# lc700x/desktop2stereo

Hardware: AMD Instinct MI355X
Metric: stereo frames/sec @1080p DepthAnything-v2-ViT-B (higher is better)
Workload: dtype bf16; 1 GPU; DepthAnything-v2-vitb bf16, 1920x1080 uint8 RGB noise frames, batch 1 per GPU, Depth Resolution 518 (model input 294x518), Full-SBS uint8 output 3840x1080, pred; parallelism=frame-sharded dp1, no data-path collective (each rank generates its own frames)

## Files before the change

desktop2stereo_amd/csrc/engine.hip:

```cpp
#include <map>
#include <string>
#include <vector>
#include <cmath>
#include <cstring>

#include "gemm.h"
#include "linear_site.h"
#include "vit_ops.h"

using namespace d2s;

namespace {

struct HostT { std::vector<float> data; std::vector<int64_t> shape; };

struct PackedW {
    void* w = nullptr;
    float* bias = nullptr;
    int N = 0, K = 0, Kpad = 0;
};

struct Layer {
    float *ln1g, *ln1b, *ln2g, *ln2b, *ls1, *ls2;
    PackedW qkv, proj, fc1, fc2;
    PackedW w8[4];
    std::vector<float> sw[4];
    PackedW qkv_ln, fc1_ln;
    float *csum_qkv = nullptr, *csum_fc1 = nullptr;
    float* deq[4] = {nullptr, nullptr, nullptr, nullptr};
    PackedW w8_ln[2];
    std::vector<float> sw_ln[2];
    float *csum8[2] = {nullptr, nullptr}, *deq_ln[2] = {nullptr, nullptr};
};

constexpr int NSITE = 6;

}

struct d2s_engine {
    d2s_model_desc d;
    int device = 0;
    int prec = D2S_PREC_BF16;
    int wprec = D2S_PREC_BF16;
    std::map<std::string, HostT> host;
    bool finalized = false;
    int h = 0, w = 0, gh = 0, gw = 0, P = 0, N = 0, Npad = 0, maxB = 0;
    uint64_t bytes = 0;
    std::vector<void*> allocs;

    PackedW patch;
    float *cls = nullptr, *pos = nullptr;
    std::vector<Layer> L;
    float *lnfg = nullptr, *lnfb = nullptr;
    struct { PackedW proj, resize, conv; PackedW proj_ln; float* csum = nullptr; } re[4];
    struct { PackedW proj, r1c1, r1c2, r2c1, r2c2; } fu[4];
    PackedW head1, head2;
    float* w3 = nullptr;
    float b3 = 0.f;

    float* resid = nullptr;
    void *lnbuf = nullptr, *qkv = nullptr, *vt = nullptr, *attn = nullptr, *mlp = nullptr, *patchA = nullptr;
    void* tapbuf[4] = {nullptr, nullptr, nullptr, nullptr};
    void* rproj[4] = {nullptr, nullptr, nullptr, nullptr};
    void* rres[4] = {nullptr, nullptr, nullptr, nullptr};
    void* feat[4] = {nullptr, nullptr, nullptr, nullptr};
    int fH[4], fW[4];
    void* scr[5] = {nullptr, nullptr, nullptr, nullptr, nullptr};
    float* splitk_ws = nullptr;
    size_t splitk_elems = 0;
    hipStream_t side = nullptr;
    hipEvent_t ev_tap[4] = {nullptr, nullptr, nullptr, nullptr}, ev_ln[4] = {nullptr, nullptr, nullptr, nullptr}, ev_side = nullptr;
    int tap_slots = 0;
    bool overlap = true;
    float* splitk_ws_side = nullptr;
    void* r1[3] = {nullptr, nullptr, nullptr};
    void* r1tmp = nullptr;
    struct TMod {
        int C = 0, sites = 0;
        float *gn_g = nullptr, *gn_b = nullptr;
        float *ln_g[2] = {nullptr, nullptr}, *ln_b[2] = {nullptr, nullptr}, *ffn_g = nullptr, *ffn_b = nullptr;
        PackedW proj_in, proj_out, kvq[2], to_out[2], ff1, ff2;
        float* ptab[2] = {nullptr, nullptr};
        void* cache[2] = {nullptr, nullptr};
        size_t ring_bytes = 0;
        PackedW kvq_ln[2], ff1_ln;
        float *csum_kvq[2] = {nullptr, nullptr}, *csum_ff1 = nullptr;
    } tm[4];
    float* tm_stats = nullptr;
    bool tm_fold = false;
    struct TSlot { int head = 0, filled = 0; };
    std::vector<TSlot> tm_slot;
    int row_ids[D2S_MAX_STREAMS] = {0};
    float* tm_hs = nullptr;
    void *tm_a = nullptr, *tm_kv = nullptr, *tm_u = nullptr, *tm_g = nullptr, *tm_out = nullptr;
    float *pre_x = nullptr, *depth_small = nullptr, *depth_post = nullptr;
    void* post_ws = nullptr;
    uint64_t post_ws_bytes = 0;
    float* ema_state = nullptr;
    int ema_init = 0;
    std::vector<int> ema_slot_init;
    bool taps = false;
    float* tap_hidden = nullptr;
    int last_batch = 0;
    bool fp8 = false, fp8_ready = false, calib = false;
    bool lnf = false;
    bool no_lnfuse = false;
    bool attn_prescaled = false;
    float* lnstats = nullptr;
    float* amax = nullptr;
    std::vector<float> act_scale;
    struct ProfRec { int cls; double flops, bytes; hipEvent_t a, b; };
    bool prof_on = false;
    std::vector<ProfRec> prof_recs;
    std::vector<hipEvent_t> prof_pool;
    size_t prof_used = 0;
};

namespace {

int dev_alloc(d2s_engine* e, void** p, size_t bytes, bool zero = false) {
    if (bytes == 0) bytes = 16;
    D2S_HIP(hipMalloc(p, bytes));
    e->allocs.push_back(*p);
    e->bytes += bytes;
    if (zero) D2S_HIP(hipMemset(*p, 0, bytes));
    return D2S_OK;
}

int dev_upload(d2s_engine* e, void** p, const void* host, size_t bytes) {
    int rc = dev_alloc(e, p, bytes);
    if (rc) return rc;
    D2S_HIP(hipMemcpy(*p, host, bytes, hipMemcpyHostToDevice));
    return D2S_OK;
}

#define RC(x) do { int _rc = (x); if (_rc != D2S_OK) return _rc; } while (0)

enum { PC_GEMM = 0, PC_CONV, PC_ATTN, PC_LN, PC_ELT, PC_PRE, PC_POST, PC_WARP, PC_N };
const char* const PC_NAMES[PC_N] = {"gemm_linear", "gemm_conv3x3", "attention", "layernorm", "elementwise", "preprocess",
                                    "post_process", "stereo_warp"};

hipEvent_t prof_event(d2s_engine* e) {
    if (e->prof_used == e->prof_pool.size()) { hipEvent_t ev; (void)hipEventCreate(&ev); e->prof_pool.push_back(ev); }
    return e->prof_pool[e->prof_used++];
}
void prof_begin(d2s_engine* e, int cls, double flops, double bytes, hipStream_t st) {
    if (!e->prof_on) return;
    d2s_engine::ProfRec r; r.cls = cls; r.flops = flops; r.bytes = bytes; r.a = prof_event(e); r.b = prof_event(e);
    (void)hipEventRecord(r.a, st);
    e->prof_recs.push_back(r);
}
void prof_end(d2s_engine* e, hipStream_t st) {
    if (!e->prof_on) return;
    (void)hipEventRecord(e->prof_recs.back().b, st);
}
#define PROF(cls, fl, by, call) do { prof_begin(e, cls, fl, by, st); int _rc = (call); prof_end(e, st); if (_rc != D2S_OK) return _rc; } while (0)

const HostT* find(d2s_engine* e, const std::string& name) {
    auto it = e->host.find(name);
    if (it == e->host.end()) { set_error("missing weight tensor: " + name); return nullptr; }
    return &it->second;
}

int upload_f32(d2s_engine* e, const std::string& name, size_t n, float** out) {
    const HostT* t = find(e, name);
    if (!t) return D2S_E_MISSING;
    if (t->data.size() != n) { set_error("weight " + name + ": wrong element count"); return D2S_E_MISSING; }
    return dev_upload(e, (void**)out, t->data.data(), n * sizeof(float));
}

int upload_linear(d2s_engine* e, LinearImage im, PackedW& out, float** csum = nullptr, std::vector<float>* sw = nullptr) {
    RC(dev_upload(e, &out.w, im.w.data(), im.w.size()));
    out.N = im.N; out.K = im.K; out.Kpad = im.Kpad;
    out.bias = nullptr;
    if (!im.bias.empty()) RC(dev_upload(e, (void**)&out.bias, im.bias.data(), im.bias.size() * sizeof(float)));
    if (csum) {
        D2S_REQUIRE(!im.csum.empty(), "upload_linear: a colsum was asked for, but no LayerNorm is folded into this linear");
        RC(dev_upload(e, (void**)csum, im.csum.data(), im.csum.size() * sizeof(float)));
    }
    if (sw) *sw = std::move(im.sw);
    return D2S_OK;
}

int pack_linear(d2s_engine* e, const std::string& wname, const std::string& bname, int N, int K, PackedW& out) {
    const HostT* w = find(e, wname);
    if (!w) return D2S_E_MISSING;
    if (w->data.size() != (size_t)N * K) { set_error("weight " + wname + ": wrong shape"); return D2S_E_MISSING; }
    const float* b = nullptr;
    if (!bname.empty()) { const HostT* bt = find(e, bname); if (!bt || bt->data.size() != (size_t)N) { set_error("bad bias " + bname); return D2S_E_MISSING; } b = bt->data.data(); }
    const float* p = w->data.data();
    return upload_linear(e, prepare_linear(e->wprec, N, K, [&](int n, int k) { return p[(size_t)n * K + k]; }, b), out);
}

int pack_conv3(d2s_engine* e, const std::string& wname, const std::string& bname, int Co, int Ci, PackedW& out) {
    const HostT* w = find(e, wname);
    if (!w) return D2S_E_MISSING;
    if (w->data.size() != (size_t)Co * Ci * 9) { set_error("weight " + wname + ": wrong shape"); return D2S_E_MISSING; }
    const float* b = nullptr;
    if (!bname.empty()) { const HostT* bt = find(e, bname); if (!bt || bt->data.size() != (size_t)Co) { set_error("bad bias " + bname); return D2S_E_MISSING; } b = bt->data.data(); }
    const float* p = w->data.data();
    return upload_linear(e, prepare_linear(e->wprec, Co, 9 * Ci, [&](int n, int k) { return p[conv3_weight_index(n, k, Ci)]; }, b), out);
}

int pack_convT(d2s_engine* e, const std::string& wname, const std::string& bname, int C, int ks, PackedW& out) {
    const HostT* w = find(e, wname);
    const HostT* bt = find(e, bname);
    if (!w || !bt) return D2S_E_MISSING;
    if (w->data.size() != (size_t)C * C * ks * ks || bt->data.size() != (size_t)C) { set_error("weight " + wname + ": wrong shape"); return D2S_E_MISSING; }
    const float* p = w->data.data();
    int N = ks * ks * C;
    std::vector<float> bias(N);
    for (int n = 0; n < N; ++n) bias[n] = bt->data[n % C];
    return upload_linear(e, prepare_linear(e->wprec, N, C, [&](int n, int k) { return p[convT_weight_index(n, k, C, ks)]; }, bias.data()), out);
}

void cubic_coeffs(float t, float c[4]) {
    const float A = -0.75f;
    auto c1 = [&](float x) { return ((A + 2.f) * x - (A + 3.f)) * x * x + 1.f; };
    auto c2 = [&](float x) { return ((A * x - 5.f * A) * x + 8.f * A) * x - 4.f * A; };
    c[0] = c2(t + 1.f); c[1] = c1(t); c[2] = c1(1.f - t); c[3] = c2(2.f - t);
}

void interp_pos(const float* pos, int grid, int D, int gh, int gw, std::vector<float>& out, double offset = 0.0) {
    out.assign((size_t)(1 + gh * gw) * D, 0.f);
    std::memcpy(out.data(), pos, D * sizeof(float));
    if (gh == grid && gw == grid) { std::memcpy(out.data() + D, pos + D, (size_t)grid * grid * D * sizeof(float)); return; }
    float sy = (float)grid / (float)gh, sx = (float)grid / (float)gw;
    if (offset != 0.0) {
        sy = (float)(1.0 / (((double)gh + offset) / (double)grid)); sx = (float)(1.0 / (((double)gw + offset) / (double)grid));
    }
    for (int oy = 0; oy < gh; ++oy) {
        float fy = sy * ((float)oy + 0.5f) - 0.5f;
        float iyf = floorf(fy);
        float cy[4]; cubic_coeffs(fy - iyf, cy);
        int iy = (int)iyf;
        for (int ox = 0; ox < gw; ++ox) {
            float fx = sx * ((float)ox + 0.5f) - 0.5f;
            float ixf = floorf(fx);
            float cx[4]; cubic_coeffs(fx - ixf, cx);
            int ix = (int)ixf;
            float* o = out.data() + (size_t)(1 + oy * gw + ox) * D;
            for (int d = 0; d < D; ++d) {
                float acc = 0.f;
                for (int a = 0; a < 4; ++a) {
                    int yy = std::min(std::max(iy - 1 + a, 0), grid - 1);
                    float row = 0.f;
                    for (int b = 0; b < 4; ++b) {
                        int xx = std::min(std::max(ix - 1 + b, 0), grid - 1);
                        row += pos[(size_t)(1 + yy * grid + xx) * D + d] * cx[b];
                    }
                    acc += row * cy[a];
                }
                o[d] = acc;
            }
        }
    }
}

GemmA plainA(const void* p, long lda) { GemmA a = {}; a.ptr = p; a.mode = A_PLAIN; a.lda = lda; return a; }
GemmA splitA(const void* p, long lda, bool split) { GemmA a = plainA(p, lda); a.bx3 = split ? 1 : 0; return a; }
GemmA convA(const void* p, int Hi, int Wi, int C, int Ho, int Wo, int stride, int relu) {
    GemmA a = {}; a.ptr = p; a.mode = A_CONV3; a.Hi = Hi; a.Wi = Wi; a.C = C; a.Ho = Ho; a.Wo = Wo; a.stride = stride; a.relu = relu; return a;
}

int gemm(d2s_engine* e, const GemmA& a, const PackedW& w, int M, const GemmEpi& ep, hipStream_t st) {
    int Kl = w.K % (e->prec == D2S_PREC_BF16 ? 8 : 4) ? w.Kpad : w.K;
    GemmEpi ep2 = ep;
    if (ep.map == MAP_ROWS) {
        ep2.part = (e->side && st == e->side) ? e->splitk_ws_side : e->splitk_ws;
        ep2.part_elems = e->splitk_elems;
    }
    PROF(a.mode == A_CONV3 ? PC_CONV : PC_GEMM, 2.0 * M * w.N * w.K, 0, launch_gemm(e->wprec, 0, a, w.w, M, w.N, Kl, w.Kpad, ep2, st));
    return D2S_OK;
}

int gemm8(d2s_engine* e, const GemmA& a, const PackedW& w, int M, const GemmEpi& ep, hipStream_t st) {
    PROF(PC_GEMM, 2.0 * M * w.N * w.K, 0, launch_gemm(D2S_PREC_FP8_OPERANDS, 0, a, w.w, M, w.N, w.K, w.Kpad, ep, st));
    return D2S_OK;
}

int conv3(d2s_engine* e, const void* in, int B, int Hi, int Wi, int C, int stride, int relu_in, const PackedW& w,
          void* out, int act, const void* res1, const void* res2, hipStream_t st) {
    int Ho = (Hi + 2 - 3) / stride + 1, Wo = (Wi + 2 - 3) / stride + 1;
    GemmA a = convA(in, Hi, Wi, C, Ho, Wo, stride, relu_in);
    GemmEpi ep = rowsE(out, OUT_T, w.N, w.bias);
    ep.act = act; ep.res1 = res1; ep.res2 = res2;
    return gemm(e, a, w, B * Ho * Wo, ep, st);
}

void window_rows(const d2s_engine::TSlot& sl, bool fold, void* ring, AttnRow& attn, CacheRow& store) {
    const bool in_attn = fold && sl.filled;
    attn = AttnRow{ring, (int16_t)sl.head, (int16_t)(sl.filled ? 32 : 1), in_attn ? sl.head : -1};
    store = CacheRow{ring, sl.filled ? sl.head : 0, sl.filled ? (in_attn ? 0 : 1) : 31};
}

int run_temporal(d2s_engine* e, int m, const void* x, void* out, int B, hipStream_t st, const void* add = nullptr) {
    d2s_engine::TMod& t = e->tm[m];
    const int C = t.C, S = B * t.sites, prec = e->prec;
    const int* ids = e->row_ids;
    const bool fold = e->tm_fold;
    int slots = 0;
    auto producer = [&](GemmEpi& ep) { if (fold) epi_ln_producer(ep, e->tm_a, e->tm_stats, &slots); };
    auto consumer = [&](GemmEpi& ep, const float* csum) { epi_ln_consumer(ep, e->tm_stats, slots, csum, 1e-5f, C); };
    void* gn_out = fold ? e->tm_out : e->tm_a;
    PROF(PC_ELT, 0, 0, launch_groupnorm(prec, x, t.gn_g, t.gn_b, gn_out, t.sites, C, 32, 1e-6f, st, B));
    {
        GemmEpi ep = rowsE(e->tm_hs, OUT_F32, C, t.proj_in.bias);
        producer(ep);
        RC(gemm(e, plainA(gn_out, C), t.proj_in, S, ep, st));
    }
    for (int a = 0; a < 2; ++a) {
        const bool folded = fold && slots >= 1 && slots <= 16;
        if (!folded) PROF(PC_LN, 0, 0, launch_layernorm(prec, e->tm_hs, t.ln_g[a], t.ln_b[a], e->tm_a, S, C, 1e-5f, 0, 0, 0, st));
        {
            GemmEpi ep = rowsE(e->tm_kv, OUT_T, 3 * C, folded ? t.kvq_ln[a].bias : nullptr);
            if (folded) consumer(ep, t.csum_kvq[a]);
            RC(gemm(e, plainA(e->tm_a, C), folded ? t.kvq_ln[a] : t.kvq[a], S, ep, st));
        }
        AttnRows attn = {};
        CacheRows store = {};
        double win_rows = 0;
        bool store_due = false;
        for (int r = 0; r < B; ++r) {
            window_rows(e->tm_slot[ids[r]], fold, (char*)t.cache[a] + (size_t)ids[r] * t.ring_bytes, attn.r[r], store.r[r]);
            win_rows += attn.r[r].Tw;
            store_due |= store.r[r].nslots > 0;
        }
        PROF(PC_ATTN, 4.0 * t.sites * win_rows * C, 0, launch_temporal_attn(prec, e->tm_kv, t.ptab[a], e->tm_out, t.sites, C, 31, B, attn, st));
        {
            GemmEpi ep = epi_residual(e->tm_hs, C, t.to_out[a].bias, nullptr);
            producer(ep);
            RC(gemm(e, plainA(e->tm_out, C), t.to_out[a], S, ep, st));
        }
        if (store_due) PROF(PC_ELT, 0, 0, launch_cache_store(prec, e->tm_kv, t.sites, C, B, store, st));
    }
    {
        const bool folded = fold && slots >= 1 && slots <= 16;
        if (!folded) PROF(PC_LN, 0, 0, launch_layernorm(prec, e->tm_hs, t.ffn_g, t.ffn_b, e->tm_a, S, C, 1e-5f, 0, 0, 0, st));
        if (folded) {
            GemmEpi ep = rowsE(e->tm_g, OUT_T, 4 * C, t.ff1_ln.bias);
            ep.act = ACT_GEGLU;
            consumer(ep, t.csum_ff1);
            RC(gemm(e, plainA(e->tm_a, C), t.ff1_ln, S, ep, st));
        } else {
            GemmEpi ep = rowsE(e->tm_u, OUT_T, 8 * C, t.ff1.bias);
            RC(gemm(e, plainA(e->tm_a, C), t.ff1, S, ep, st));
            PROF(PC_ELT, 0, 0, launch_geglu(prec, e->tm_u, e->tm_g, S, 4 * C, st));
        }
    }
    {
        GemmEpi ep = epi_residual(e->tm_hs, C, t.ff2.bias, nullptr);
        if (fold) epi_ln_producer(ep, e->tm_a, nullptr, nullptr);
        RC(gemm(e, plainA(e->tm_g, 4 * C), t.ff2, S, ep, st));
    }
    const void* a_out = e->tm_a;
    if (!fold) {
        if (prec == D2S_PREC_BF16) PROF(PC_ELT, 0, 0, launch_cast_f32(prec, e->tm_hs, e->tm_a, (long)S * C, st));
        else a_out = e->tm_hs;
    }
    {
        GemmEpi ep = rowsE(out, OUT_T, C, t.proj_out.bias);
        ep.res1 = x; ep.res2 = add;
        RC(gemm(e, plainA(a_out, C), t.proj_out, S, ep, st));
    }
    return D2S_OK;
}

int neck_proj(d2s_engine* e, int i, int B, hipStream_t st, bool fold) {
    const d2s_model_desc& d = e->d;
    const int D = d.hidden, Mp = B * e->P, c = d.neck[i];
    if (!fold) return gemm(e, plainA(e->tapbuf[i], D), e->re[i].proj, Mp, rowsE(e->rproj[i], OUT_T, c, e->re[i].proj.bias), st);
    GemmEpi ep = rowsE(e->rproj[i], OUT_T, c, e->re[i].proj_ln.bias);
    epi_ln_consumer(ep, e->lnstats, e->tap_slots, e->re[i].csum, d.ln_eps, D);
    const int skip = epi_tap_fold_rows(ep, B, e->N, e->P);
    return gemm(e, plainA((const bf16_t*)e->lnbuf + (size_t)skip * D, D), e->re[i].proj_ln, skip ? Mp : B * e->N, ep, st);
}

int neck_rest(d2s_engine* e, int i, int B, hipStream_t st) {
    const d2s_model_desc& d = e->d;
    const int F = d.fusion, gh = e->gh, gw = e->gw, Mp = B * e->P, c = d.neck[i];
    const void* src = e->rproj[i];
    int Hs = gh, Ws = gw;
    if (i < 2) {
        int ks = i == 0 ? 4 : 2;
        RC(gemm(e, plainA(e->rproj[i], c), e->re[i].resize, Mp, epi_convT(e->rres[i], c, e->re[i].resize.bias, gh, gw, ks), st));
        src = e->rres[i]; Hs = gh * ks; Ws = gw * ks;
    } else if (i == 3) {
        RC(conv3(e, e->rproj[i], B, gh, gw, c, 2, 0, e->re[i].resize, e->rres[i], ACT_NONE, nullptr, nullptr, st));
        src = e->rres[i]; Hs = (gh - 1) / 2 + 1; Ws = (gw - 1) / 2 + 1;
    }
    if (d.temporal && i == 2) { RC(run_temporal(e, 0, src, e->rres[2], B, st)); src = e->rres[2]; }
    if (d.temporal && i == 3) { RC(run_temporal(e, 1, src, e->scr[0], B, st)); src = e->scr[0]; }
    RC(conv3(e, src, B, Hs, Ws, c, 1, 0, e->re[i].conv, e->feat[i], ACT_NONE, nullptr, nullptr, st));
    if (i < 3) {
        const int idx = 3 - i;
        RC(conv3(e, e->feat[i], B, Hs, Ws, F, 1, 1, e->fu[idx].r1c1, e->r1tmp, ACT_NONE, nullptr, nullptr, st));
        RC(conv3(e, e->r1tmp, B, Hs, Ws, F, 1, 1, e->fu[idx].r1c2, e->r1[i], ACT_NONE, e->feat[i], nullptr, st));
    }
    return D2S_OK;
}

int forward(d2s_engine* e, const float* x, float* depth, int B, hipStream_t st) {
    const d2s_model_desc& d = e->d;
    const int D = d.hidden, N = e->N, P = e->P, M = B * N, Mp = B * P, prec = e->prec;
    const int F = d.fusion;
    const PrecRules pr = prec_rules(d.precision);
    const bool use_side = e->overlap && e->side != nullptr && !e->prof_on;
    if (e->fp8 && !e->fp8_ready && !e->calib) {
        set_error("D2S_PREC_FP8 engine: activation scales are not set, call d2s_engine_calibrate first");
        return D2S_E_STATE;
    }
    if (x) PROF(PC_ELT, 0, 0, launch_patchify(prec, x, e->patchA, B, e->h, e->w, d.patch, e->patch.Kpad, e->cls, e->pos, e->resid, N, D, st));
    {
        RC(gemm(e, plainA(e->patchA, e->patch.Kpad), e->patch, Mp, epi_patch_embed(e->resid, D, e->patch.bias, e->pos, P, N), st));
    }
    if (e->taps) D2S_HIP(hipMemcpyAsync(e->tap_hidden, e->resid, (size_t)N * D * 4, hipMemcpyDeviceToDevice, st));
    int tap_i = 0;
    const bool f8 = e->fp8 && !e->calib;
    const bool f8a = f8 && pr.e4m3_attn;
    const bool x3 = e->wprec == D2S_PREC_BF16X3;
    static EnvInt lnf_pp{"D2S_LNF_PP", 1};
    const bool pp_fold = lnf_pp.get() && e->lnf && e->wprec == D2S_PREC_BF16 && !e->calib && !e->taps && D % 256 == 0 && D <= 1024 &&
                         gemm_pp_min_tiles() > 0 && (long)cdiv(M, 256) * (D / 256) >= gemm_pp_min_tiles();
    const bool lnf = (pr.ln_folds(D2S_LIN_FC1) && !e->no_lnfuse && !e->calib && B <= (x3 ? 8 : 3)) || pp_fold;
    int ln_slots = 0;
    const bool tap_fold = lnf && pr.ln_folds(D2S_LIN_NECK_PROJ) && (B == 1 || pp_fold);
    bool tap_folded[4] = {false, false, false, false};
    int pending_ln = -1;
    for (int l = 0; l < d.layers; ++l) {
        const Layer& ly = e->L[l];
        const float* sa = f8 ? &e->act_scale[(size_t)l * NSITE] : nullptr;
        float* am = e->calib ? e->amax + (size_t)l * NSITE : nullptr;
        const bool ln1_folded = lnf && l > 0 && ln_slots <= 16 && pr.ln_folds(D2S_LIN_QKV);
        if (!ln1_folded) PROF(PC_LN, 0, 0, launch_layernorm(prec, e->resid, ly.ln1g, ly.ln1b, e->lnbuf, M, D, d.ln_eps, 0, 0, 0, st, f8a ? 1.0f / sa[0] : 0.f, x3));
        if (am) RC(launch_amax(prec, e->lnbuf, (long)M * D, am + 0, st));
        {
            GemmEpi ep = epi_qkv(e->qkv, qkv_out_type(f8, x3), D, ln1_folded ? (f8a ? ly.w8_ln[0].bias : ly.qkv_ln.bias) : ly.qkv.bias, e->vt, N, e->Npad, d.heads);
            if (ln1_folded) epi_ln_consumer(ep, e->lnstats, ln_slots, f8a ? ly.csum8[0] : ly.csum_qkv, d.ln_eps, D);
            if (f8a) { ep.deq = ln1_folded ? ly.deq_ln[0] : ly.deq[0]; RC(gemm8(e, plainA(e->lnbuf, D), ln1_folded ? ly.w8_ln[0] : ly.w8[0], M, ep, st)); }
            else RC(gemm(e, splitA(e->lnbuf, D, x3), ln1_folded ? ly.qkv_ln : ly.qkv, M, ep, st));
        }
        PROF(PC_ATTN, 4.0 * B * d.heads * (double)N * N * 64, 0,
             launch_attention(x3 ? D2S_PREC_BF16X3 : prec, e->qkv, e->vt, e->attn, B, N, e->Npad, d.heads, st, f8a ? 1.0f / sa[1] : 0.f, e->attn_prescaled));
        if (am) RC(launch_amax(prec, e->attn, (long)M * D, am + 1, st));
        {
            if (pending_ln >= 0) { D2S_HIP(hipStreamWaitEvent(st, e->ev_ln[pending_ln], 0)); pending_ln = -1; }
            GemmEpi ep = epi_residual(e->resid, D, ly.proj.bias, ly.ls1);
            if (lnf) epi_ln_producer(ep, e->lnbuf, e->lnstats, &ln_slots, x3, f8 ? 1.0f / sa[4] : 0.f);
            if (f8a) { ep.deq = ly.deq[1]; RC(gemm8(e, plainA(e->attn, D), ly.w8[1], M, ep, st)); }
            else RC(gemm(e, splitA(e->attn, D, x3), ly.proj, M, ep, st));
        }
        const bool ln2_folded = lnf && ln_slots <= 16;
        if (!ln2_folded) PROF(PC_LN, 0, 0, launch_layernorm(prec, e->resid, ly.ln2g, ly.ln2b, e->lnbuf, M, D, d.ln_eps, 0, 0, 0, st, f8 ? 1.0f / sa[2] : 0.f, x3));
        if (am) RC(launch_amax(D2S_PREC_FP32, e->resid, (long)M * D, am + 4, st));
        if (am) RC(launch_amax(prec, e->lnbuf, (long)M * D, am + 2, st));
        {
            GemmEpi ep = epi_fc1(e->mlp, fc1_out_type(x3), d.mlp, ln2_folded ? (f8 ? ly.w8_ln[1].bias : ly.fc1_ln.bias) : ly.fc1.bias);
            if (ln2_folded) epi_ln_consumer(ep, e->lnstats, ln_slots, f8 ? ly.csum8[1] : ly.csum_fc1, d.ln_eps, D);
            if (f8) { ep.deq = ln2_folded ? ly.deq_ln[1] : ly.deq[2]; ep.out_qscale = 1.0f / sa[3]; RC(gemm8(e, plainA(e->lnbuf, D), ln2_folded ? ly.w8_ln[1] : ly.w8[2], M, ep, st)); }
            else RC(gemm(e, splitA(e->lnbuf, D, x3), ln2_folded ? ly.fc1_ln : ly.fc1, M, ep, st));
        }
        if (am) RC(launch_amax(prec, e->mlp, (long)M * d.mlp, am + 3, st));
        {
            GemmEpi ep = epi_residual(e->resid, D, ly.fc2.bias, ly.ls2);
            if (lnf && (l + 1 < d.layers || tap_fold) && pr.ln_folds(D2S_LIN_FC2)) epi_ln_producer(ep, e->lnbuf, e->lnstats, &ln_slots, x3, f8 ? 1.0f / sa[5] : 0.f);
            if (f8) { ep.deq = ly.deq[3]; RC(gemm8(e, plainA(e->mlp, d.mlp), ly.w8[3], M, ep, st)); }
            else RC(gemm(e, splitA(e->mlp, d.mlp, x3), ly.fc2, M, ep, st));
        }
        if (am) RC(launch_amax(D2S_PREC_FP32, e->resid, (long)M * D, am + 5, st));
        if (e->taps) D2S_HIP(hipMemcpyAsync(e->tap_hidden + (size_t)(l + 1) * N * D, e->resid, (size_t)N * D * 4, hipMemcpyDeviceToDevice, st));
        if (tap_i < 4 && l + 1 == d.out_indices[tap_i]) {
            const bool fold = tap_fold && ln_slots <= 16;
            tap_folded[tap_i] = fold;
            e->tap_slots = ln_slots;
            if (!fold) PROF(PC_LN, 0, 0, launch_layernorm(prec, e->resid, e->lnfg, e->lnfb, e->tapbuf[tap_i], Mp, D, d.ln_eps, P, N, 1, st));
            if (use_side && (tap_i < 3 || d.temporal)) {
                D2S_HIP(hipEventRecord(e->ev_tap[tap_i], st));
                D2S_HIP(hipStreamWaitEvent(e->side, e->ev_tap[tap_i], 0));
                RC(neck_proj(e, tap_i, B, e->side, fold));
                if (fold) { D2S_HIP(hipEventRecord(e->ev_ln[tap_i], e->side)); pending_ln = tap_i; }
                RC(neck_rest(e, tap_i, B, e->side));
            } else {
                RC(neck_proj(e, tap_i, B, st, fold));
            }
            ++tap_i;
        }
    }
    for (int i = 0; i < 4; ++i)
        if (!(use_side && (i < 3 || d.temporal))) RC(neck_rest(e, i, B, st));
    if (use_side) {
        D2S_HIP(hipEventRecord(e->ev_side, e->side));
        D2S_HIP(hipStreamWaitEvent(st, e->ev_side, 0));
    }
    void *X = e->scr[0], *Y = e->scr[1], *Z = e->scr[2];
    void* fused = nullptr;
    bool fold1 = false;
    GemmA c1a = {};
    int Hc = 0, Wc = 0;
    for (int idx = 0; idx < 4; ++idx) {
        int mi = 3 - idx;
        void* m = e->feat[mi];
        Hc = e->fH[mi]; Wc = e->fW[mi];
        const void* hcur = idx == 0 ? m : fused;
        RC(conv3(e, hcur, B, Hc, Wc, F, 1, 1, e->fu[idx].r2c1, X, ACT_NONE, nullptr, nullptr, st));
        RC(conv3(e, X, B, Hc, Wc, F, 1, 1, e->fu[idx].r2c2, Z, ACT_NONE, hcur, nullptr, st));
        int Ho, Wo;
        if (idx < 3) { Ho = e->fH[mi - 1]; Wo = e->fW[mi - 1]; } else { Ho = Hc * 2; Wo = Wc * 2; }
        void* pout = e->scr[3 + (idx & 1)];
        const void* next_r1 = idx < 3 ? e->r1[2 - idx] : nullptr;
        RC(gemm(e, plainA(Z, F), e->fu[idx].proj, B * Hc * Wc, rowsE(X, OUT_T, F, e->fu[idx].proj.bias), st));
        if (d.temporal && idx < 2) {
            PROF(PC_ELT, 0, 0, launch_bilinear_nhwc(prec, X, pout, B, Hc, Wc, Ho, Wo, F, st));
            void* alt = e->scr[3 + ((idx + 1) & 1)];
            RC(run_temporal(e, 2 + idx, pout, alt, B, st, next_r1));
            pout = alt;
        } else {
            if (idx == 3) {
                c1a = convA(X, Ho, Wo, F, Ho, Wo, 1, 0);
                c1a.ups = 1; c1a.Hs = Hc; c1a.Ws = Wc; c1a.usy = linear_scale(Hc, Ho, true); c1a.usx = linear_scale(Wc, Wo, true);
                GemmEpi ep1 = rowsE(Y, OUT_T, e->head1.N, e->head1.bias);
                fold1 = conv3_upsample_ok(e->wprec, 0, c1a, B * Ho * Wo, e->head1.N, e->head1.K, e->head1.Kpad, ep1);
            }
            if (!fold1) PROF(PC_ELT, 0, 0, launch_bilinear_nhwc(prec, X, pout, B, Hc, Wc, Ho, Wo, F, st, next_r1));
        }
        fused = pout; Hc = Ho; Wc = Wo;
    }
    void* c1out = X;
    void* up2 = Y;
    if (fold1) {
        c1out = Y; up2 = X;
        GemmEpi ep1 = rowsE(c1out, OUT_T, e->head1.N, e->head1.bias);
        PROF(PC_CONV, 2.0 * B * Hc * Wc * e->head1.N * e->head1.K, 0, launch_gemm(e->wprec, 0, c1a, e->head1.w, B * Hc * Wc, e->head1.N, e->head1.K, e->head1.Kpad, ep1, st));
    } else {
        RC(conv3(e, fused, B, Hc, Wc, F, 1, 0, e->head1, c1out, ACT_NONE, nullptr, nullptr, st));
    }
    {
        const int Mh = B * e->h * e->w, Nh = d.head_hidden;
        const int bn = Nh <= 32 ? 32 : 64;
        const bool fused_tail = Nh <= 64 && (long)cdiv(Mh, 256) * cdiv(Nh, bn) >= 224;
        GemmA a = convA(up2, e->h, e->w, F / 2, e->h, e->w, 1, 0);
        GemmEpi ep = rowsE(depth, OUT_F32, 1, e->head2.bias);
        ep.map = MAP_HEAD; ep.scale = e->w3; ep.head_b3 = e->b3; ep.head_max_depth = d.max_depth;
        GemmA au = a;
        au.ptr = c1out; au.ups = 1; au.Hs = Hc; au.Ws = Wc; au.usy = linear_scale(Hc, e->h, true); au.usx = linear_scale(Wc, e->w, true);
        const bool ups = fused_tail && conv3_upsample_ok(e->wprec, head_tile(bn), au, Mh, Nh, e->head2.K, e->head2.Kpad, ep);
        if (!ups) PROF(PC_ELT, 0, 0, launch_bilinear_nhwc(prec, c1out, up2, B, Hc, Wc, e->h, e->w, F / 2, st));
        if (fused_tail) {
            PROF(PC_CONV, 2.0 * Mh * Nh * e->head2.K, 0, launch_gemm(e->wprec, head_tile(bn), ups ? au : a, e->head2.w, Mh, Nh, e->head2.K, e->head2.Kpad, ep, st));
        } else {
            RC(conv3(e, up2, B, e->h, e->w, F / 2, 1, 0, e->head2, Z, ACT_RELU, nullptr, nullptr, st));
            PROF(PC_ELT, 0, 0, launch_head_final(prec, Z, e->w3, e->b3, d.max_depth, depth, (long)B * e->h * e->w, d.head_hidden, st));
        }
    }
    if (d.temporal) {
        for (int r = 0; r < B; ++r) {
            d2s_engine::TSlot& sl = e->tm_slot[e->row_ids[r]];
            if (sl.filled) sl.head = (sl.head + 1) % 31;
            sl.filled = 1;
        }
    }
    e->last_batch = B;
    return D2S_OK;
}

}

extern "C" int d2s_engine_create(const d2s_model_desc* desc, int device_id, d2s_engine** out) {
    D2S_REQUIRE(desc && out, "null pointer");
    D2S_REQUIRE(desc->hidden > 0 && desc->heads > 0 && desc->hidden == desc->heads * 64, "head_dim must be 64");
    D2S_REQUIRE(desc->layers > 0 && desc->patch > 0 && desc->pos_grid > 0 && desc->fusion % 8 == 0, "bad model desc");
    D2S_REQUIRE(desc->precision == D2S_PREC_FP32 || desc->precision == D2S_PREC_BF16 || desc->precision == D2S_PREC_FP8 ||
                desc->precision == D2S_PREC_BF16X3 || desc->precision == D2S_PREC_FP8_MLP, "bad precision");
    for (int i = 0; i < 4; ++i) D2S_REQUIRE(desc->neck[i] % 8 == 0 && desc->out_indices[i] >= 1 && desc->out_indices[i] <= desc->layers, "bad neck / out_indices");
    D2S_REQUIRE(desc->head_hidden % 4 == 0 && desc->mlp % 8 == 0, "bad head_hidden / mlp");
    D2S_REQUIRE(desc->max_depth >= 0.f && !(desc->temporal && desc->max_depth > 0.f),
                "max_depth must be >= 0, and 0 for a Video-Depth-Anything engine (its head ends in ReLU, dpt_temporal.py:136)");
    D2S_ON_DEVICE(device_id);
    d2s_engine* e = new d2s_engine();
    e->d = *desc; e->device = device_id;
    const PrecRules pr = prec_rules(desc->precision);
    e->fp8 = pr.e4m3;
    e->no_lnfuse = env_int("D2S_NO_LNFUSE", 0) != 0;
    e->lnf = pr.ln_folds(D2S_LIN_FC1) && !pr.e4m3 && !e->no_lnfuse;
    e->prec = pr.act;
    e->wprec = pr.w;
    e->attn_prescaled = e->prec == D2S_PREC_BF16;
    e->taps = env_int("D2S_TAPS", 0) != 0;
    *out = e;
    return D2S_OK;
}

extern "C" int d2s_engine_set_weight(d2s_engine* e, const char* name, const float* host, const int64_t* shape, int ndim) {
    D2S_REQUIRE(e && name && host && shape && ndim >= 1 && ndim <= 4, "bad argument");
    if (e->finalized) { set_error("d2s_engine_set_weight after finalize"); return D2S_E_STATE; }
    HostT t;
    size_t n = 1;
    for (int i = 0; i < ndim; ++i) { D2S_REQUIRE(shape[i] > 0, "bad shape"); n *= (size_t)shape[i]; t.shape.push_back(shape[i]); }
    t.data.assign(host, host + n);
    e->host[name] = std::move(t);
    return D2S_OK;
}

extern "C" int d2s_engine_finalize(d2s_engine* e, int h, int w, int max_batch) {
    D2S_REQUIRE(e, "null engine");
    if (e->finalized) { set_error("engine already finalized"); return D2S_E_STATE; }
    const d2s_model_desc& d = e->d;
    D2S_REQUIRE(h > 0 && w > 0 && h % d.patch == 0 && w % d.patch == 0 && max_batch >= 1, "h, w must be patch multiples");
    D2S_REQUIRE(!d.temporal || max_batch <= D2S_MAX_STREAMS, "a Video-Depth-Anything engine has at most D2S_MAX_STREAMS (32) stream slots: max_batch too large");
    D2S_ON_DEVICE(e->device);
    const int D = d.hidden, F = d.fusion;
    e->h = h; e->w = w; e->gh = h / d.patch; e->gw = w / d.patch; e->P = e->gh * e->gw; e->N = e->P + 1;
    e->Npad = (e->N + 63) / 64 * 64; e->maxB = max_batch;
    const int N = e->N, P = e->P, B = max_batch;
    const size_t es = elem_size(e->prec);
    std::string pe = "backbone.embeddings.";
    RC(pack_linear(e, pe + "patch_embeddings.projection.weight", pe + "patch_embeddings.projection.bias", D, 3 * d.patch * d.patch, e->patch));
    RC(upload_f32(e, pe + "cls_token", D, &e->cls));
    {
        const HostT* pt = find(e, pe + "position_embeddings");
        if (!pt) return D2S_E_MISSING;
        if (pt->data.size() != (size_t)(d.pos_grid * d.pos_grid + 1) * D) { set_error("position_embeddings: wrong shape"); return D2S_E_MISSING; }
        std::vector<float> pos;
        interp_pos(pt->data.data(), d.pos_grid, D, e->gh, e->gw, pos, d.temporal ? 0.1 : 0.0);
        RC(dev_alloc(e, (void**)&e->pos, pos.size() * 4));
        D2S_HIP(hipMemcpy(e->pos, pos.data(), pos.size() * 4, hipMemcpyHostToDevice));
    }
    e->L.resize(d.layers);
    for (int l = 0; l < d.layers; ++l) {
        std::string p = "backbone.encoder.layer." + std::to_string(l) + ".";
        Layer& ly = e->L[l];
        RC(upload_f32(e, p + "norm1.weight", D, &ly.ln1g)); RC(upload_f32(e, p + "norm1.bias", D, &ly.ln1b));
        RC(upload_f32(e, p + "norm2.weight", D, &ly.ln2g)); RC(upload_f32(e, p + "norm2.bias", D, &ly.ln2b));
        RC(upload_f32(e, p + "layer_scale1.lambda1", D, &ly.ls1)); RC(upload_f32(e, p + "layer_scale2.lambda1", D, &ly.ls2));
        const HostT *wq = find(e, p + "attention.attention.query.weight"), *wk = find(e, p + "attention.attention.key.weight"),
                    *wv = find(e, p + "attention.attention.value.weight"), *bq = find(e, p + "attention.attention.query.bias"),
                    *bk = find(e, p + "attention.attention.key.bias"), *bv = find(e, p + "attention.attention.value.bias");
        if (!wq || !wk || !wv || !bq || !bk || !bv) return D2S_E_MISSING;
        for (const HostT* t : {wq, wk, wv}) if (t->data.size() != (size_t)D * D) { set_error("qkv weight: wrong shape"); return D2S_E_MISSING; }
        std::vector<float> bias(3 * D);
        for (int i = 0; i < D; ++i) { bias[i] = bq->data[i]; bias[D + i] = bk->data[i]; bias[2 * D + i] = bv->data[i]; }
        std::vector<float> wq_scaled;
        if (e->attn_prescaled) {
            wq_scaled.resize(wq->data.size());
            for (size_t i = 0; i < wq_scaled.size(); ++i) wq_scaled[i] = wq->data[i] * ATTN_SCALE_LOG2E;
            for (int i = 0; i < D; ++i) bias[i] *= ATTN_SCALE_LOG2E;
        }
        const float* ws[3] = {e->attn_prescaled ? wq_scaled.data() : wq->data.data(), wk->data.data(), wv->data.data()};
        auto qkv_at = [&](int n, int k) { return ws[n / D][(size_t)(n % D) * D + k]; };
        RC(upload_linear(e, prepare_linear(e->wprec, 3 * D, D, qkv_at, bias.data()), ly.qkv));
        RC(pack_linear(e, p + "attention.output.dense.weight", p + "attention.output.dense.bias", D, D, ly.proj));
        RC(pack_linear(e, p + "mlp.fc1.weight", p + "mlp.fc1.bias", d.mlp, D, ly.fc1));
        RC(pack_linear(e, p + "mlp.fc2.weight", p + "mlp.fc2.bias", D, d.mlp, ly.fc2));
        const HostT *g1 = find(e, p + "norm1.weight"), *bn1 = find(e, p + "norm1.bias"), *g2 = find(e, p + "norm2.weight"), *bn2 = find(e, p + "norm2.bias");
        const HostT *wo = find(e, p + "attention.output.dense.weight"), *w1 = find(e, p + "mlp.fc1.weight"), *b1 = find(e, p + "mlp.fc1.bias"),
                    *w2 = find(e, p + "mlp.fc2.weight");
        if (!g1 || !bn1 || !g2 || !bn2 || !wo || !w1 || !b1 || !w2) return D2S_E_MISSING;
        auto fc1_at = [&](int n, int k) { return w1->data[(size_t)n * D + k]; };
        if (e->lnf) {
            RC(upload_linear(e, prepare_linear(e->wprec, 3 * D, D, qkv_at, bias.data(), g1->data.data(), bn1->data.data()), ly.qkv_ln, &ly.csum_qkv));
            RC(upload_linear(e, prepare_linear(e->wprec, d.mlp, D, fc1_at, b1->data.data(), g2->data.data(), bn2->data.data()), ly.fc1_ln, &ly.csum_fc1));
        }
        if (e->fp8) {
            const int e8 = D2S_PREC_FP8_OPERANDS;
            RC(upload_linear(e, prepare_linear(e8, 3 * D, D, qkv_at, nullptr), ly.w8[0], nullptr, &ly.sw[0]));
            RC(upload_linear(e, prepare_linear(e8, D, D, [&](int n, int k) { return wo->data[(size_t)n * D + k]; }, nullptr), ly.w8[1], nullptr, &ly.sw[1]));
            RC(upload_linear(e, prepare_linear(e8, d.mlp, D, fc1_at, nullptr), ly.w8[2], nullptr, &ly.sw[2]));
            RC(upload_linear(e, prepare_linear(e8, D, d.mlp, [&](int n, int k) { return w2->data[(size_t)n * d.mlp + k]; }, nullptr), ly.w8[3], nullptr, &ly.sw[3]));
            const PackedW* w16[4] = {&ly.qkv, &ly.proj, &ly.fc1, &ly.fc2};
            for (int i = 0; i < 4; ++i) {
                ly.w8[i].bias = w16[i]->bias;
                RC(dev_alloc(e, (void**)&ly.deq[i], (size_t)ly.w8[i].N * sizeof(float), true));
            }
            RC(upload_linear(e, prepare_linear(e8, 3 * D, D, qkv_at, bias.data(), g1->data.data(), bn1->data.data()), ly.w8_ln[0], &ly.csum8[0], &ly.sw_ln[0]));
            RC(dev_alloc(e, (void**)&ly.deq_ln[0], (size_t)3 * D * sizeof(float), true));
            RC(upload_linear(e, prepare_linear(e8, d.mlp, D, fc1_at, b1->data.data(), g2->data.data(), bn2->data.data()), ly.w8_ln[1], &ly.csum8[1], &ly.sw_ln[1]));
            RC(dev_alloc(e, (void**)&ly.deq_ln[1], (size_t)d.mlp * sizeof(float), true));
        }
    }
    if (e->fp8) {
        RC(dev_alloc(e, (void**)&e->amax, (size_t)d.layers * NSITE * sizeof(float), true));
        e->act_scale.assign((size_t)d.layers * NSITE, 0.f);
    }
    RC(upload_f32(e, "backbone.layernorm.weight", D, &e->lnfg));
    RC(upload_f32(e, "backbone.layernorm.bias", D, &e->lnfb));
    for (int i = 0; i < 4; ++i) {
        std::string p = "neck.reassemble_stage.layers." + std::to_string(i) + ".";
        int c = d.neck[i];
        RC(pack_linear(e, p + "projection.weight", p + "projection.bias", c, D, e->re[i].proj));
        if (i == 0) RC(pack_convT(e, p + "resize.weight", p + "resize.bias", c, 4, e->re[i].resize));
        if (i == 1) RC(pack_convT(e, p + "resize.weight", p + "resize.bias", c, 2, e->re[i].resize));
        if (i == 3) RC(pack_conv3(e, p + "resize.weight", p + "resize.bias", c, c, e->re[i].resize));
        RC(pack_conv3(e, "neck.convs." + std::to_string(i) + ".weight", "", F, c, e->re[i].conv));
    }
    if (e->lnf) {
        const HostT *gf = find(e, "backbone.layernorm.weight"), *bf = find(e, "backbone.layernorm.bias");
        if (!gf || !bf) return D2S_E_MISSING;
        for (int i = 0; i < 4; ++i) {
            std::string p = "neck.reassemble_stage.layers." + std::to_string(i) + ".projection.";
            const HostT *wt = find(e, p + "weight"), *bt = find(e, p + "bias");
            if (!wt || !bt) return D2S_E_MISSING;
            RC(upload_linear(e, prepare_linear(e->wprec, d.neck[i], D, [&](int n, int k) { return wt->data[(size_t)n * D + k]; }, bt->data.data(),
                                               gf->data.data(), bf->data.data()), e->re[i].proj_ln, &e->re[i].csum));
        }
    }
    for (int i = 0; i < 4; ++i) {
        std::string p = "neck.fusion_stage.layers." + std::to_string(i) + ".";
        RC(pack_linear(e, p + "projection.weight", p + "projection.bias", F, F, e->fu[i].proj));
        RC(pack_conv3(e, p + "residual_layer1.convolution1.weight", p + "residual_layer1.convolution1.bias", F, F, e->fu[i].r1c1));
        RC(pack_conv3(e, p + "residual_layer1.convolution2.weight", p + "residual_layer1.convolution2.bias", F, F, e->fu[i].r1c2));
        RC(pack_conv3(e, p + "residual_layer2.convolution1.weight", p + "residual_layer2.convolution1.bias", F, F, e->fu[i].r2c1));
        RC(pack_conv3(e, p + "residual_layer2.convolution2.weight", p + "residual_layer2.convolution2.bias", F, F, e->fu[i].r2c2));
    }
    RC(pack_conv3(e, "head.conv1.weight", "head.conv1.bias", F / 2, F, e->head1));
    RC(pack_conv3(e, "head.conv2.weight", "head.conv2.bias", d.head_hidden, F / 2, e->head2));
    RC(upload_f32(e, "head.conv3.weight", d.head_hidden, &e->w3));
    { const HostT* b3 = find(e, "head.conv3.bias"); if (!b3) return D2S_E_MISSING; e->b3 = b3->data[0]; }
    const size_t M = (size_t)B * N, Mp = (size_t)B * P;
    RC(dev_alloc(e, (void**)&e->resid, M * D * 4));
    RC(dev_alloc(e, &e->lnbuf, M * D * es));
    if (e->lnf || e->fp8) RC(dev_alloc(e, (void**)&e->lnstats, (size_t)(D / 16 + 1) * M * 2 * sizeof(float)));
    RC(dev_alloc(e, &e->qkv, M * 3 * D * es));
    RC(dev_alloc(e, &e->vt, (size_t)B * D * e->Npad * es, true));
    RC(dev_alloc(e, &e->attn, M * D * es));
    RC(dev_alloc(e, &e->mlp, M * d.mlp * es));
    RC(dev_alloc(e, &e->patchA, Mp * e->patch.Kpad * es, true));
    const int gh = e->gh, gw = e->gw;
    e->fH[0] = gh * 4; e->fW[0] = gw * 4; e->fH[1] = gh * 2; e->fW[1] = gw * 2; e->fH[2] = gh; e->fW[2] = gw;
    e->fH[3] = (gh - 1) / 2 + 1; e->fW[3] = (gw - 1) / 2 + 1;
    for (int i = 0; i < 4; ++i) {
        RC(dev_alloc(e, &e->tapbuf[i], Mp * D * es));
        RC(dev_alloc(e, &e->rproj[i], Mp * d.neck[i] * es));
        RC(dev_alloc(e, &e->rres[i], (size_t)B * e->fH[i] * e->fW[i] * d.neck[i] * es));
        RC(dev_alloc(e, &e->feat[i], (size_t)B * e->fH[i] * e->fW[i] * F * es));
    }
    size_t scr_elems = std::max({(size_t)64 * gh * gw * F, (size_t)h * w * (F / 2), (size_t)h * w * d.head_hidden}) * B;
    for (int i = 0; i < 5; ++i) RC(dev_alloc(e, &e->scr[i], scr_elems * es));
    e->splitk_elems = (size_t)B * 16 * e->fH[2] * e->fW[2] * std::max(F, d.neck[3]);
    RC(dev_alloc(e, (void**)&e->splitk_ws, (e->splitk_elems + GEMM_PART_CTR_WORDS) * 4, true));
    for (int i = 0; i < 3; ++i) RC(dev_alloc(e, &e->r1[i], (size_t)B * e->fH[i] * e->fW[i] * F * es));
    RC(dev_alloc(e, &e->r1tmp, (size_t)B * e->fH[0] * e->fW[0] * F * es));
    RC(dev_alloc(e, (void**)&e->splitk_ws_side, (e->splitk_elems + GEMM_PART_CTR_WORDS) * 4, true));
    e->overlap = env_int("D2S_NO_OVERLAP", 0) == 0;
    if (e->overlap) {
        D2S_HIP(hipStreamCreateWithFlags(&e->side, hipStreamNonBlocking));
        for (int i = 0; i < 4; ++i) D2S_HIP(hipEventCreateWithFlags(&e->ev_tap[i], hipEventDisableTiming));
        for (int i = 0; i < 4; ++i) D2S_HIP(hipEventCreateWithFlags(&e->ev_ln[i], hipEventDisableTiming));
        D2S_HIP(hipEventCreateWithFlags(&e->ev_side, hipEventDisableTiming));
    }
    if (d.temporal) {
        const int tC[4] = {d.neck[2], d.neck[3], F, F};
        const int tS[4] = {e->fH[2] * e->fW[2], e->fH[3] * e->fW[3], e->fH[2] * e->fW[2], e->fH[1] * e->fW[1]};
        size_t sc_max = 0, max_sites = 0;
        e->tm_fold = prec_rules(d.precision).ln_folds(D2S_LIN_TM_KVQ) && env_int("D2S_VDA_FUSE", 1) != 0;
        for (int m = 0; m < 4; ++m) {
            d2s_engine::TMod& t = e->tm[m];
            t.C = tC[m]; t.sites = tS[m];
            max_sites = std::max(max_sites, (size_t)t.sites);
            const int C = t.C;
            D2S_REQUIRE(C % 32 == 0 && C <= 1024, "temporal module channels must be a multiple of 32 (GroupNorm) and <= 1024");
            sc_max = std::max(sc_max, (size_t)t.sites * C);
            std::string p = "head.motion_modules." + std::to_string(m) + ".temporal_transformer.";
            std::string b = p + "transformer_blocks.0.";
            RC(upload_f32(e, p + "norm.weight", C, &t.gn_g)); RC(upload_f32(e, p + "norm.bias", C, &t.gn_b));
            RC(pack_linear(e, p + "proj_in.weight", p + "proj_in.bias", C, C, t.proj_in));
            RC(pack_linear(e, p + "proj_out.weight", p + "proj_out.bias", C, C, t.proj_out));
            std::vector<float> pe((size_t)32 * C);
            for (int i = 0; i < C / 2; ++i) {
                float div = expf((float)(2 * i) * (float)(-std::log(10000.0) / C));
                for (int pos = 0; pos < 32; ++pos) { pe[(size_t)pos * C + 2 * i] = sinf((float)pos * div); pe[(size_t)pos * C + 2 * i + 1] = cosf((float)pos * div); }
            }
            for (int a = 0; a < 2; ++a) {
                std::string q = b + "attention_blocks." + std::to_string(a) + ".";
                RC(upload_f32(e, b + "norms." + std::to_string(a) + ".weight", C, &t.ln_g[a]));
                RC(upload_f32(e, b + "norms." + std::to_string(a) + ".bias", C, &t.ln_b[a]));
                const HostT *wq = find(e, q + "to_q.weight"), *wk = find(e, q + "to_k.weight"), *wv = find(e, q + "to_v.weight");
                if (!wq || !wk || !wv) return D2S_E_MISSING;
                for (const HostT* w3 : {wq, wk, wv}) if (w3->data.size() != (size_t)C * C) { set_error("to_q/to_k/to_v: wrong shape"); return D2S_E_MISSING; }
                const float* kvq[3] = {wk->data.data(), wv->data.data(), wq->data.data()};
                auto kvq_at = [&](int n, int k) { return kvq[n / C][(size_t)(n % C) * C + k]; };
                RC(upload_linear(e, prepare_linear(e->wprec, 3 * C, C, kvq_at, nullptr), t.kvq[a]));
                std::vector<float> pt((size_t)32 * 3 * C);
                for (int j = 0; j < 32; ++j)
                    for (int n = 0; n < 3 * C; ++n) {
                        const float* wr = kvq[n / C] + (size_t)(n % C) * C;
                        double acc = 0.0;
                        for (int k = 0; k < C; ++k) acc += (double)pe[(size_t)j * C + k] * (double)wr[k];
                        pt[(size_t)j * 3 * C + n] = (float)acc;
                    }
                RC(dev_alloc(e, (void**)&t.ptab[a], pt.size() * 4));
                D2S_HIP(hipMemcpy(t.ptab[a], pt.data(), pt.size() * 4, hipMemcpyHostToDevice));
                RC(pack_linear(e, q + "to_out.0.weight", q + "to_out.0.bias", C, C, t.to_out[a]));
                t.ring_bytes = (size_t)31 * t.sites * 2 * C * es;
                RC(dev_alloc(e, &t.cache[a], (size_t)B * t.ring_bytes, true));
                if (e->tm_fold) {
                    const HostT *g = find(e, b + "norms." + std::to_string(a) + ".weight"), *bt = find(e, b + "norms." + std::to_string(a) + ".bias");
                    if (!g || !bt) return D2S_E_MISSING;
                    RC(upload_linear(e, prepare_linear(e->wprec, 3 * C, C, kvq_at, nullptr, g->data.data(), bt->data.data()), t.kvq_ln[a], &t.csum_kvq[a]));
                }
            }
            RC(upload_f32(e, b + "ff_norm.weight", C, &t.ffn_g)); RC(upload_f32(e, b + "ff_norm.bias", C, &t.ffn_b));
            RC(pack_linear(e, b + "ff.net.0.proj.weight", b + "ff.net.0.proj.bias", 8 * C, C, t.ff1));
            RC(pack_linear(e, b + "ff.net.2.weight", b + "ff.net.2.bias", C, 4 * C, t.ff2));
            if (e->tm_fold) {
                const HostT *g = find(e, b + "ff_norm.weight"), *bt = find(e, b + "ff_norm.bias"), *w1 = find(e, b + "ff.net.0.proj.weight"),
                            *b1 = find(e, b + "ff.net.0.proj.bias");
                if (!g || !bt || !w1 || !b1) return D2S_E_MISSING;
                const float* w1p = w1->data.data();
                auto orig = [C](int n) { return geglu_row(n, C); };
                std::vector<float> b1p((size_t)8 * C);
                for (int n = 0; n < 8 * C; ++n) b1p[n] = b1->data[orig(n)];
                RC(upload_linear(e, prepare_linear(e->wprec, 8 * C, C, [&](int n, int k) { return w1p[(size_t)orig(n) * C + k]; }, b1p.data(),
                                                   g->data.data(), bt->data.data()), t.ff1_ln, &t.csum_ff1));
            }
        }
        sc_max *= (size_t)B; max_sites *= (size_t)B;
        e->tm_slot.assign(B, d2s_engine::TSlot());
        e->ema_slot_init.assign(B, 0);
        if (e->tm_fold) RC(dev_alloc(e, (void**)&e->tm_stats, (size_t)17 * max_sites * 2 * sizeof(float)));
        RC(dev_alloc(e, (void**)&e->tm_hs, sc_max * 4));
        RC(dev_alloc(e, &e->tm_a, sc_max * es)); RC(dev_alloc(e, &e->tm_out, sc_max * es));
        RC(dev_alloc(e, &e->tm_kv, sc_max * 3 * es));
        RC(dev_alloc(e, &e->tm_u, sc_max * 8 * es)); RC(dev_alloc(e, &e->tm_g, sc_max * 4 * es));
    }
    e->host.clear();
    RC(dev_alloc(e, (void**)&e->pre_x, (size_t)B * 3 * h * w * 4));
    RC(dev_alloc(e, (void**)&e->depth_small, (size_t)B * h * w * 4));
    RC(dev_alloc(e, (void**)&e->depth_post, (size_t)B * h * w * 4));
    e->post_ws_bytes = d2s_post_process_workspace(B, h, w);
    RC(dev_alloc(e, &e->post_ws, e->post_ws_bytes));
    RC(dev_alloc(e, (void**)&e->ema_state, (size_t)(d.temporal ? B : 1) * h * w * 4));
    if (e->taps) RC(dev_alloc(e, (void**)&e->tap_hidden, (size_t)(d.layers + 1) * N * D * 4));
    D2S_HIP(hipDeviceSynchronize());
    e->finalized = true;
    return D2S_OK;
}

extern "C" int d2s_engine_destroy(d2s_engine* e) {
    if (!e) return D2S_OK;
    D2S_ON_DEVICE(e->device);
    if (e->side) (void)hipStreamSynchronize(e->side);
    for (int i = 0; i < 4; ++i) if (e->ev_tap[i]) (void)hipEventDestroy(e->ev_tap[i]);
    for (int i = 0; i < 4; ++i) if (e->ev_ln[i]) (void)hipEventDestroy(e->ev_ln[i]);
    if (e->ev_side) (void)hipEventDestroy(e->ev_side);
    if (e->side) (void)hipStreamDestroy(e->side);
    for (void* p : e->allocs) (void)hipFree(p);
    delete e;
    return D2S_OK;
}

extern "C" int d2s_engine_memory(const d2s_engine* e, uint64_t* bytes) {
    D2S_REQUIRE(e && bytes, "null pointer");
    *bytes = e->bytes;
    return D2S_OK;
}

namespace {
int resolve_streams(d2s_engine* e, int batch, const int* stream_ids) {
    if (!e->d.temporal) {
        D2S_REQUIRE(!stream_ids, "stream_ids on an engine that is not a Video-Depth-Anything engine: its batch rows are not streams");
        return D2S_OK;
    }
    uint32_t seen = 0;
    for (int r = 0; r < batch; ++r) {
        const int id = stream_ids ? stream_ids[r] : r;
        if (id < 0 || id >= e->maxB) { set_error("stream id " + std::to_string(id) + " out of range: the engine has " + std::to_string(e->maxB) + " stream slot(s)"); return D2S_E_INVALID; }
        if (seen >> id & 1u) { set_error("stream id " + std::to_string(id) + " named twice in one call"); return D2S_E_INVALID; }
        seen |= 1u << id;
    }
    for (int r = 0; r < batch; ++r) e->row_ids[r] = stream_ids ? stream_ids[r] : r;
    return D2S_OK;
}
}

extern "C" int d2s_model_forward_streams(d2s_engine* e, const float* x, float* depth, int batch, const int* stream_ids, void* stream) {
    D2S_REQUIRE(e && x && depth, "null pointer");
    if (!e->finalized) { set_error("d2s_model_forward before d2s_engine_finalize"); return D2S_E_STATE; }
    D2S_REQUIRE(batch >= 1 && batch <= e->maxB, "batch exceeds max_batch");
    RC(resolve_streams(e, batch, stream_ids));
    D2S_ON_DEVICE(e->device);
    return forward(e, x, depth, batch, (hipStream_t)stream);
}

extern "C" int d2s_model_forward(d2s_engine* e, const float* x, float* depth, int batch, void* stream) {
    return d2s_model_forward_streams(e, x, depth, batch, nullptr, stream);
}

extern "C" int d2s_engine_calibrate(d2s_engine* e, const float* x, int batch, void* stream) {
    D2S_REQUIRE(e && x, "null pointer");
    if (!e->finalized) { set_error("d2s_engine_calibrate before d2s_engine_finalize"); return D2S_E_STATE; }
    D2S_REQUIRE(e->fp8, "d2s_engine_calibrate: not a D2S_PREC_FP8 engine");
    D2S_REQUIRE(batch >= 1 && batch <= e->maxB && !e->d.temporal, "bad batch (or a Video-Depth-Anything engine)");
    D2S_ON_DEVICE(e->device);
    hipStream_t st = (hipStream_t)stream;
    const int L = e->d.layers;
    D2S_HIP(hipMemsetAsync(e->amax, 0, (size_t)L * NSITE * sizeof(float), st));
// ... 228 lines not shown
```

Baseline: 889.5 stereo frames/s.

## Double-buffer FC2 layernorm outputs to relax side-stream neck projection waits

Adds two ping-pong LN buffers and stats arrays that the FC2 epilogue writes by layer parity. The next layer's QKV and the neck projection read from them. The main stream now waits on the side-stream neck_proj event only when the same parity buffer is about to be overwritten, two layers later, rather than before the next proj GEMM. This lets the tap neck projections overlap with more backbone work, at the cost of extra device memory and more complex buffer-ownership logic.

After: 885.1 stereo frames/s. No clear change (-0.5%).

```diff
diff --git a/desktop2stereo_amd/csrc/engine.hip b/desktop2stereo_amd/csrc/engine.hip
--- a/desktop2stereo_amd/csrc/engine.hip
+++ b/desktop2stereo_amd/csrc/engine.hip
@@ -107,6 +107,8 @@
     bool no_lnfuse = false;
     bool attn_prescaled = false;
     float* lnstats = nullptr;
+    void* lnbuf_f[2] = {nullptr, nullptr};
+    float* lnstats_f[2] = {nullptr, nullptr};
     float* amax = nullptr;
     std::vector<float> act_scale;
     struct ProfRec { int cls; double flops, bytes; hipEvent_t a, b; };
@@ -117,6 +119,12 @@
 };
 
 namespace {
+
+struct LnSet { void* buf; float* stats; int idx; };
+static inline LnSet fc2_ln_set(const d2s_engine* e, int l) {
+    if (!e->lnbuf_f[0]) return {e->lnbuf, e->lnstats, 0};
+    return {e->lnbuf_f[l & 1], e->lnstats_f[l & 1], l & 1};
+}
 
 int dev_alloc(d2s_engine* e, void** p, size_t bytes, bool zero = false) {
     if (bytes == 0) bytes = 16;
@@ -371,9 +379,10 @@
     const int D = d.hidden, Mp = B * e->P, c = d.neck[i];
     if (!fold) return gemm(e, plainA(e->tapbuf[i], D), e->re[i].proj, Mp, rowsE(e->rproj[i], OUT_T, c, e->re[i].proj.bias), st);
     GemmEpi ep = rowsE(e->rproj[i], OUT_T, c, e->re[i].proj_ln.bias);
-    epi_ln_consumer(ep, e->lnstats, e->tap_slots, e->re[i].csum, d.ln_eps, D);
+    const LnSet ls = fc2_ln_set(e, d.out_indices[i] - 1);
+    epi_ln_consumer(ep, ls.stats, e->tap_slots, e->re[i].csum, d.ln_eps, D);
     const int skip = epi_tap_fold_rows(ep, B, e->N, e->P);
-    return gemm(e, plainA((const bf16_t*)e->lnbuf + (size_t)skip * D, D), e->re[i].proj_ln, skip ? Mp : B * e->N, ep, st);
+    return gemm(e, plainA((const bf16_t*)ls.buf + (size_t)skip * D, D), e->re[i].proj_ln, skip ? Mp : B * e->N, ep, st);
 }
 
 int neck_rest(d2s_engine* e, int i, int B, hipStream_t st) {
@@ -426,25 +435,25 @@
     int ln_slots = 0;
     const bool tap_fold = lnf && pr.ln_folds(D2S_LIN_NECK_PROJ) && (B == 1 || pp_fold);
     bool tap_folded[4] = {false, false, false, false};
-    int pending_ln = -1;
+    int pending_ln[2] = {-1, -1};
     for (int l = 0; l < d.layers; ++l) {
         const Layer& ly = e->L[l];
         const float* sa = f8 ? &e->act_scale[(size_t)l * NSITE] : nullptr;
         float* am = e->calib ? e->amax + (size_t)l * NSITE : nullptr;
         const bool ln1_folded = lnf && l > 0 && ln_slots <= 16 && pr.ln_folds(D2S_LIN_QKV);
+        const LnSet in1 = ln1_folded ? fc2_ln_set(e, l - 1) : LnSet{e->lnbuf, e->lnstats, 0};
         if (!ln1_folded) PROF(PC_LN, 0, 0, launch_layernorm(prec, e->resid, ly.ln1g, ly.ln1b, e->lnbuf, M, D, d.ln_eps, 0, 0, 0, st, f8a ? 1.0f / sa[0] : 0.f, x3));
-        if (am) RC(launch_amax(prec, e->lnbuf, (long)M * D, am + 0, st));
+        if (am) RC(launch_amax(prec, in1.buf, (long)M * D, am + 0, st));
         {
             GemmEpi ep = epi_qkv(e->qkv, qkv_out_type(f8, x3), D, ln1_folded ? (f8a ? ly.w8_ln[0].bias : ly.qkv_ln.bias) : ly.qkv.bias, e->vt, N, e->Npad, d.heads);
-            if (ln1_folded) epi_ln_consumer(ep, e->lnstats, ln_slots, f8a ? ly.csum8[0] : ly.csum_qkv, d.ln_eps, D);
-            if (f8a) { ep.deq = ln1_folded ? ly.deq_ln[0] : ly.deq[0]; RC(gemm8(e, plainA(e->lnbuf, D), ln1_folded ? ly.w8_ln[0] : ly.w8[0], M, ep, st)); }
-            else RC(gemm(e, splitA(e->lnbuf, D, x3), ln1_folded ? ly.qkv_ln : ly.qkv, M, ep, st));
+            if (ln1_folded) epi_ln_consumer(ep, in1.stats, ln_slots, f8a ? ly.csum8[0] : ly.csum_qkv, d.ln_eps, D);
+            if (f8a) { ep.deq = ln1_folded ? ly.deq_ln[0] : ly.deq[0]; RC(gemm8(e, plainA(in1.buf, D), ln1_folded ? ly.w8_ln[0] : ly.w8[0], M, ep, st)); }
+            else RC(gemm(e, splitA(in1.buf, D, x3), ln1_folded ? ly.qkv_ln : ly.qkv, M, ep, st));
         }
         PROF(PC_ATTN, 4.0 * B * d.heads * (double)N * N * 64, 0,
              launch_attention(x3 ? D2S_PREC_BF16X3 : prec, e->qkv, e->vt, e->attn, B, N, e->Npad, d.heads, st, f8a ? 1.0f / sa[1] : 0.f, e->attn_prescaled));
         if (am) RC(launch_amax(prec, e->attn, (long)M * D, am + 1, st));
         {
-            if (pending_ln >= 0) { D2S_HIP(hipStreamWaitEvent(st, e->ev_ln[pending_ln], 0)); pending_ln = -1; }
             GemmEpi ep = epi_residual(e->resid, D, ly.proj.bias, ly.ls1);
             if (lnf) epi_ln_producer(ep, e->lnbuf, e->lnstats, &ln_slots, x3, f8 ? 1.0f / sa[4] : 0.f);
             if (f8a) { ep.deq = ly.deq[1]; RC(gemm8(e, plainA(e->attn, D), ly.w8[1], M, ep, st)); }
@@ -463,7 +472,9 @@
         if (am) RC(launch_amax(prec, e->mlp, (long)M * d.mlp, am + 3, st));
         {
             GemmEpi ep = epi_residual(e->resid, D, ly.fc2.bias, ly.ls2);
-            if (lnf && (l + 1 < d.layers || tap_fold) && pr.ln_folds(D2S_LIN_FC2)) epi_ln_producer(ep, e->lnbuf, e->lnstats, &ln_slots, x3, f8 ? 1.0f / sa[5] : 0.f);
+            const LnSet out2 = fc2_ln_set(e, l);
+            if (pending_ln[out2.idx] >= 0) { D2S_HIP(hipStreamWaitEvent(st, e->ev_ln[pending_ln[out2.idx]], 0)); pending_ln[out2.idx] = -1; }
+            if (lnf && (l + 1 < d.layers || tap_fold) && pr.ln_folds(D2S_LIN_FC2)) epi_ln_producer(ep, out2.buf, out2.stats, &ln_slots, x3, f8 ? 1.0f / sa[5] : 0.f);
             if (f8) { ep.deq = ly.deq[3]; RC(gemm8(e, plainA(e->mlp, d.mlp), ly.w8[3], M, ep, st)); }
             else RC(gemm(e, splitA(e->mlp, d.mlp, x3), ly.fc2, M, ep, st));
         }
@@ -478,7 +489,7 @@
                 D2S_HIP(hipEventRecord(e->ev_tap[tap_i], st));
                 D2S_HIP(hipStreamWaitEvent(e->side, e->ev_tap[tap_i], 0));
                 RC(neck_proj(e, tap_i, B, e->side, fold));
-                if (fold) { D2S_HIP(hipEventRecord(e->ev_ln[tap_i], e->side)); pending_ln = tap_i; }
+                if (fold) { D2S_HIP(hipEventRecord(e->ev_ln[tap_i], e->side)); pending_ln[fc2_ln_set(e, l).idx] = tap_i; }
                 RC(neck_rest(e, tap_i, B, e->side));
             } else {
                 RC(neck_proj(e, tap_i, B, st, fold));
@@ -718,7 +729,8 @@
     const size_t M = (size_t)B * N, Mp = (size_t)B * P;
     RC(dev_alloc(e, (void**)&e->resid, M * D * 4));
     RC(dev_alloc(e, &e->lnbuf, M * D * es));
-    if (e->lnf || e->fp8) RC(dev_alloc(e, (void**)&e->lnstats, (size_t)(D / 16 + 1) * M * 2 * sizeof(float)));
+    const size_t stats_bytes = (size_t)(D / 16 + 1) * M * 2 * sizeof(float);
+    if (e->lnf || e->fp8) RC(dev_alloc(e, (void**)&e->lnstats, stats_bytes));
     RC(dev_alloc(e, &e->qkv, M * 3 * D * es));
     RC(dev_alloc(e, &e->vt, (size_t)B * D * e->Npad * es, true));
     RC(dev_alloc(e, &e->attn, M * D * es));
@@ -741,6 +753,8 @@
     RC(dev_alloc(e, &e->r1tmp, (size_t)B * e->fH[0] * e->fW[0] * F * es));
     RC(dev_alloc(e, (void**)&e->splitk_ws_side, (e->splitk_elems + GEMM_PART_CTR_WORDS) * 4, true));
     e->overlap = env_int("D2S_NO_OVERLAP", 0) == 0;
+    if (e->overlap && (e->lnf || e->fp8))
+        for (int i = 0; i < 2; ++i) { RC(dev_alloc(e, &e->lnbuf_f[i], M * D * es)); RC(dev_alloc(e, (void**)&e->lnstats_f[i], stats_bytes)); }
     if (e->overlap) {
         D2S_HIP(hipStreamCreateWithFlags(&e->side, hipStreamNonBlocking));
         for (int i = 0; i < 4; ++i) D2S_HIP(hipEventCreateWithFlags(&e->ev_tap[i], hipEventDisableTiming));
```
